# Rigelyon/ThatsMyFace

Hardware: AMD Instinct MI355X
Metric: Mpixels/s embed+extract, 4K RGB batch, 1/2/4/8 MI355X; % HBM roofline (higher is better)
Workload: dtype f64+f32 (u8 I/O)

## Files before the change

thatsmyface_amd/csrc/tmfwm_internal.h:

```cpp
#pragma once
#include <hip/hip_runtime.h>
#include <stdint.h>

#include <vector>

#include "../../include/tmfwm.h"
#include "tmfwm_sizes.h"
#include "tmfwm_tile_plan.h"

namespace tmf {

constexpr uint32_t kListShards = 2048, kShardStride = 16;

__host__ __device__ inline uint32_t shard_base(uint32_t s, uint32_t rows, uint32_t nbw)
{
    const uint32_t q = rows / kListShards, r = rows % kListShards;
    return (uint32_t)(((uint64_t)s * q + (s < r ? s : r)) * nbw);
}

struct EmbedArgs {
    const uint8_t *src;
    uint8_t *dst;
    const uint8_t *wm;
    int64_t wm_stride;
    int64_t nframes;
    int64_t frame_stride;
    int H, W, block, nbh, nbw, strips_per_row;
    int aligned;
    double alpha;
    uint32_t *fb_list;
    uint32_t *fb_count;
    uint32_t *fb_bad;
    uint32_t *slow_list;
    uint32_t *slow_count;
    uint32_t *slow_shards;
    float *key_out;
    int64_t key_stride;
};

struct ExtractArgs {
    const uint8_t *wsrc;
    const uint8_t *osrc;
    uint8_t *out;
    int64_t nframes;
    int64_t frame_stride;
    int64_t tile_stride;
    int H, W, block, nbh, nbw, strips_per_row;
    int aligned;
    float alpha32;
    uint32_t *fb_list;
    uint32_t *fb_count;
    uint32_t *fb_bad;
    uint32_t *slow_list;
    uint32_t *slow_count;
    uint32_t *slow_shards;
};

struct KeyedArgs {
    const uint8_t *src;
    const float *key;
    float *key_out;
    uint8_t *out;
    int64_t nframes;
    int64_t frame_stride;
    int64_t tile_stride;
    int64_t key_stride;
    int H, W, block, nbh, nbw, strips_per_row;
    int aligned;
    float alpha32;
    uint32_t *fb_list;
    uint32_t *fb_count;
    uint32_t *fb_bad;
    uint32_t *slow_list;
    uint32_t *slow_count;
    uint32_t *slow_shards;
};

struct EdgeArgs {
    const uint8_t *src;
    uint8_t *dst;
    int64_t frame_stride;
    int H, W, core_h, core_w, edge_w;
};

int report(int code, const char *fmt, ...);
void clear_error();
int check_frames(int64_t n, int32_t H, int32_t W, int64_t stride, int32_t block);

int64_t count_chunks(int64_t nframes, int H, int W, int block);
int embed_device_async(const uint8_t *src, int64_t n, int H, int W, int64_t stride, const uint8_t *tile, int64_t tile_stride,
                       int block, double alpha, uint8_t *dst, hipStream_t st, uint32_t *sink, int route = TMFWM_ROUTE_HYBRID);
int extract_device_async(const uint8_t *wsrc, const uint8_t *osrc, int64_t n, int H, int W, int64_t stride, int block,
                         double alpha, uint8_t *out, hipStream_t st, uint32_t *sink, int route = TMFWM_ROUTE_HYBRID);
int sum_sink(const uint32_t *sink, int64_t nchunks, int64_t *lapack);


constexpr int64_t kMaxGridY = 65535;

template <class Launch>
inline hipError_t for_frame_slices(int64_t nframes, Launch launch)
{
    for (int64_t f0 = 0; f0 < nframes; f0 += kMaxGridY) launch(f0, nframes - f0 < kMaxGridY ? nframes - f0 : kMaxGridY);
    return hipGetLastError();
}

inline unsigned list_grid(int64_t rows) { return (unsigned)(rows < (int64_t)kListShards ? rows : (int64_t)kListShards); }

template <class Args>
inline hipError_t launch_strips(Args a, int bpw, void (*strip)(Args), void (*list)(Args), hipStream_t st)
{
    if (a.nframes > kMaxGridY) return hipErrorInvalidValue;
    a.strips_per_row = (a.nbw + bpw - 1) / bpw;
    hipLaunchKernelGGL(strip, dim3((unsigned)((int64_t)a.strips_per_row * a.nbh), (unsigned)a.nframes), dim3(64), 0, st, a);
    if (list && a.slow_list) hipLaunchKernelGGL(list, dim3(list_grid(a.nframes * a.nbh)), dim3(64), 0, st, a);
    return hipGetLastError();
}

hipError_t launch_embed(const EmbedArgs &a, hipStream_t st);
hipError_t launch_embed_key_strips(const EmbedArgs &a, hipStream_t st);
bool embed_key_fused(int block);
hipError_t launch_embed_rank1(EmbedArgs a, hipStream_t st);
bool rank1_block(int block);
bool embed_defers(int block);
hipError_t launch_edges(const uint8_t *src, uint8_t *dst, int64_t nframes, int H, int W, int64_t frame_stride, int block, hipStream_t st);
hipError_t launch_extract(const ExtractArgs &a, hipStream_t st);
hipError_t launch_rgb_to_ycbcr(const uint8_t *rgb, int64_t npix, float *ycc, hipStream_t st);
hipError_t launch_rgb_to_ycbcr_f32(const float *rgb, int64_t npix, float *ycc, hipStream_t st);
hipError_t launch_ycbcr_to_rgb(const void *ycc, int dtype, int64_t npix, uint8_t *rgb, hipStream_t st);
hipError_t launch_dct2d_blocks(float *blocks, int64_t nb, int block, int inverse, hipStream_t st);
hipError_t launch_embed_fixup(const EmbedArgs &a, const uint32_t *list, const uint32_t *count, int64_t max_entries, hipStream_t st);
hipError_t launch_extract_fixup(const ExtractArgs &a, const uint32_t *list, const uint32_t *count, int64_t max_entries, hipStream_t st);
template <int B>
hipError_t embed_fixup_b(const EmbedArgs &a, const uint32_t *list, const uint32_t *count, int64_t max_entries, hipStream_t st);
template <int B>
hipError_t embed_key_fixup_b(const EmbedArgs &a, const uint32_t *list, const uint32_t *count, int64_t max_entries, hipStream_t st);
template <int B>
hipError_t embed_key_strips_b(const EmbedArgs &a, hipStream_t st);
template <int B>
hipError_t extract_fixup_b(const ExtractArgs &a, const uint32_t *list, const uint32_t *count, int64_t max_entries, hipStream_t st);
template <int B>
hipError_t sigma1_fixup_b(const KeyedArgs &a, const uint32_t *list, const uint32_t *count, int64_t max_entries, hipStream_t st);
template <int B>
hipError_t extract_keyed_fixup_b(const KeyedArgs &a, const uint32_t *list, const uint32_t *count, int64_t max_entries, hipStream_t st);
hipError_t launch_sigma1_map(const KeyedArgs &a, hipStream_t st);
hipError_t launch_extract_keyed(const KeyedArgs &a, hipStream_t st);
hipError_t launch_sigma1_fixup(const KeyedArgs &a, const uint32_t *list, const uint32_t *count, int64_t max_entries, hipStream_t st);
hipError_t launch_extract_keyed_fixup(const KeyedArgs &a, const uint32_t *list, const uint32_t *count, int64_t max_entries,
                                      hipStream_t st);
hipError_t launch_list_all(uint32_t *list, uint32_t *count, int64_t n, hipStream_t st);
hipError_t launch_pack_rgbx(const uint8_t *src4, int64_t sstride, uint8_t *dst3, int64_t dstride, int64_t n, int H, int W,
                            hipStream_t st);
hipError_t launch_unpack_rgbx(const uint8_t *src3, int64_t sstride, uint8_t *dst4, int64_t dstride, int64_t n, int H, int W,
                              hipStream_t st);
hipError_t launch_lapack_svd_blocks(const float *D, int64_t nb, int block, float *U, float *S, float *Vt, int want_v, int32_t *info,
                                    hipStream_t st);
hipError_t launch_lapack_nrm2(const double *x, int64_t nvec, int n, int inc, double *out, hipStream_t st);
hipError_t launch_svd_blocks(const float *D, int64_t nb, int block, float *U, float *S, float *Vt, int32_t *sweeps, hipStream_t st);
struct ResamplePlan {
    int ih = 0, iw = 0, oh = 0, ow = 0, y_first = 0, y_last = 0;
    bool need_h = false, need_v = false;
    ResampleAxis h, v;
    void build(int in_h, int in_w, int out_h, int out_w);
    int rows() const { return y_last - y_first; }
    size_t tmp_bytes() const { return need_h ? (size_t)rows() * ow : 0; }
    std::vector<int> pack() const;
};

hipError_t launch_resize_lanczos(const uint8_t *in, const ResamplePlan &plan, const int *tables, uint8_t *tmp, uint8_t *out,
                                 int ldo, hipStream_t st);
constexpr int64_t kResizeGroup = 1024;
size_t resize_tmp_bytes(const ResamplePlan &plan, int64_t n);
hipError_t launch_resize_lanczos_batch(const uint8_t *in, int64_t in_stride, int64_t n, const ResamplePlan &plan, const int *tables,
                                       uint8_t *tmp, uint8_t *out, int ldo, int64_t out_stride, hipStream_t st);
hipError_t launch_tiles_ragged(const TileJob *jobs, int64_t n, const int *tables, uint8_t *scratch, int64_t h_items,
                               int64_t v_items, hipStream_t st);
hipError_t launch_synth(uint64_t seed, int64_t frame0, int64_t nframes, int64_t frame_bytes, uint8_t *out, hipStream_t st);

}
```

thatsmyface_amd/csrc/tmfwm_kernels.hip:

```cpp
#include "tmfwm_blocks.h"
#include "tmfwm_passes.h"

namespace tmf {

extern template __global__ void embed_kernel<8, false>(EmbedArgs);
extern template __global__ void embed_kernel<8, true>(EmbedArgs);

template <int B, bool LIST = false>
__global__ __launch_bounds__(64, (B > 8 ? 2 : kExtract8Waves)) void extract_kernel(ExtractArgs a)
{
    constexpr int L = Geo<B>::L, BPW = Geo<B>::BPW, LD = B + 1;
    __shared__ float lds[BPW * B * LD];
    const int lane = threadIdx.x & 63, g = lane / L, q = lane % L;
    float *tile = lds + g * B * LD;
    if constexpr (LIST) {
        const uint32_t per_frame = (uint32_t)a.nbh * (uint32_t)a.nbw, rows = (uint32_t)a.nframes * (uint32_t)a.nbh;
        for (uint32_t s = blockIdx.x; s < kListShards; s += gridDim.x) {
          const uint32_t n = a.slow_shards[s * kShardStride], base = shard_base(s, rows, (uint32_t)a.nbw);
          if (n != 0 && lane == 0) atomicAdd(a.slow_count, n);
          for (uint32_t t0 = 0; t0 < n; t0 += BPW) {
            StripPos pos;
            pos.valid = t0 + g < n;
            const uint32_t id = pos.valid ? a.slow_list[base + t0 + g] : 0u;
            pos.frame = id / per_frame;
            const uint32_t rem = id % per_frame;
            pos.bi = (int)(rem / (uint32_t)a.nbw);
            pos.bj = (int)(rem % (uint32_t)a.nbw);
            float sw, so;
            bool ok;
            extract_sigmas<B, kListPowerIters>(a, pos, tile, q, sw, so, ok);
            if (pos.valid && q == 0) {
                if (ok) a.out[pos.frame * a.tile_stride + (int64_t)pos.bi * a.nbw + pos.bj] = extract_byte(sw, so, a.alpha32);
                else a.fb_list[atomicAdd(a.fb_count, 1u)] = id;
            }
            __syncthreads();
          }
        }
    } else {
        const StripPos pos = strip_pos<B>(a.strips_per_row, a.nbw);
        float sw, so;
        bool ok;
        extract_sigmas<B, kPowerIters>(a, pos, tile, q, sw, so, ok);
        if (!pos.valid || q != 0) return;
        const uint32_t id = (uint32_t)(((int64_t)blockIdx.y * a.nbh + pos.bi) * a.nbw + pos.bj);
        if (!ok) {
            if (a.slow_list) {
                const uint32_t row = blockIdx.y * (uint32_t)a.nbh + (uint32_t)pos.bi, s = row % kListShards;
                a.slow_list[shard_base(s, (uint32_t)a.nframes * (uint32_t)a.nbh, (uint32_t)a.nbw) +
                            atomicAdd(a.slow_shards + s * kShardStride, 1u)] = id;
            }
            else a.fb_list[atomicAdd(a.fb_count, 1u)] = id;
            return;
        }
        a.out[pos.frame * a.tile_stride + (int64_t)pos.bi * a.nbw + pos.bj] = extract_byte(sw, so, a.alpha32);
    }
}

__global__ __launch_bounds__(256) void edge_roundtrip_kernel(EdgeArgs a)
{
    edge_roundtrip_pixel(a, (int64_t)blockIdx.x * blockDim.x + threadIdx.x, blockIdx.y * a.frame_stride);
}

__global__ __launch_bounds__(256) void rgb_to_ycbcr_kernel(const uint8_t *__restrict__ rgb, int64_t npix, float *__restrict__ ycc)
{
    const int64_t p = (int64_t)blockIdx.x * blockDim.x + threadIdx.x;
    if (p >= npix) return;
    const uint32_t r = rgb[3 * p], g = rgb[3 * p + 1], b = rgb[3 * p + 2];
    float cbs, crs;
    chroma(r, g, b, cbs, crs);
    ycc[3 * p] = luma(r, g, b);
    ycc[3 * p + 1] = cbs;
    ycc[3 * p + 2] = crs;
}

__global__ __launch_bounds__(256) void rgb_to_ycbcr_f32_kernel(const float *__restrict__ rgb, int64_t npix, float *__restrict__ ycc)
{
    const int64_t p = (int64_t)blockIdx.x * blockDim.x + threadIdx.x;
    if (p >= npix) return;
    colour_fwd_f32(rgb[3 * p], rgb[3 * p + 1], rgb[3 * p + 2], ycc[3 * p], ycc[3 * p + 1], ycc[3 * p + 2]);
}

template <typename T>
__global__ __launch_bounds__(256) void ycbcr_to_rgb_kernel(const T *__restrict__ ycc, int64_t npix, uint8_t *__restrict__ rgb)
{
    const int64_t p = (int64_t)blockIdx.x * blockDim.x + threadIdx.x;
    if (p >= npix) return;
    uint32_t R8, G8, B8;
    colour_inv_t<T>(ycc[3 * p], ycc[3 * p + 1], ycc[3 * p + 2], R8, G8, B8);
    rgb[3 * p] = (uint8_t)R8;
    rgb[3 * p + 1] = (uint8_t)G8;
    rgb[3 * p + 2] = (uint8_t)B8;
}

template <int B, bool INVERSE>
__global__ __launch_bounds__(64) void dct2d_blocks_kernel(float *blocks, int64_t nblocks)
{
    constexpr int L = Geo<B>::L, R = Geo<B>::R, BPW = Geo<B>::BPW, LD = B + 1;
    __shared__ float lds[BPW * B * LD];
    const int lane = threadIdx.x & 63, g = lane / L, q = lane % L;
    const int64_t blk = (int64_t)blockIdx.x * BPW + g;
    const bool valid = blk < nblocks;
    float x[R][B];
#pragma unroll
    for (int r = 0; r < R; ++r)
#pragma unroll
        for (int c = 0; c < B; ++c) x[r][c] = valid && real_row<B>(q, r) ? blocks[blk * B * B + (q * R + r) * B + c] : 0.0f;
    dct2d_rows_layout<B, INVERSE>(x, lds + g * B * LD, q);
    if (valid)
#pragma unroll
        for (int r = 0; r < R; ++r)
            if (real_row<B>(q, r))
#pragma unroll
                for (int c = 0; c < B; ++c) blocks[blk * B * B + (q * R + r) * B + c] = x[r][c];
}

template <int B>
__global__ __launch_bounds__(64) void svd_blocks_kernel(const float *__restrict__ D, int64_t nblocks, float *__restrict__ U,
                                                        float *__restrict__ S, float *__restrict__ Vt, int32_t *__restrict__ sweeps)
{
    constexpr int L = Geo<B>::L, R = Geo<B>::R, BPW = Geo<B>::BPW;
    constexpr int SD = (kScratchFloats<B, L> + 1) / 2;
    __shared__ double norms[BPW * SD];
    const int lane = threadIdx.x & 63, g = lane / L, q = lane % L;
    const int64_t blk = (int64_t)blockIdx.x * BPW + g;
    const bool valid = blk < nblocks;
    float x[R][B];
#pragma unroll
    for (int r = 0; r < R; ++r)
#pragma unroll
        for (int c = 0; c < B; ++c) x[r][c] = valid && real_row<B>(q, r) ? D[blk * B * B + (q * R + r) * B + c] : 0.0f;
    double A[R][B], V[R][B];
    int nsw = svd3<B, L>(x, A, V, q, NoStamp{}, norms + g * SD);
    double sig[B];
    float Uf[R][B], Vf[R][B];
#pragma unroll
    for (int k = 0; k < B; ++k) sig[k] = cdot_part<R, B>(A, k, k);
#pragma unroll
    for (int k = 0; k < B; ++k) {
        sig[k] = __builtin_sqrt(group_sum<L>(sig[k]));
        const double inv = 1.0 / sig[k];
#pragma unroll
        for (int r = 0; r < R; ++r) {
            Uf[r][k] = sig[k] == 0.0 ? 0.0f : (float)(A[r][k] * inv);
            Vf[r][k] = (float)V[r][k];
        }
    }
    bool zero = true;
#pragma unroll
    for (int k = 0; k < B; ++k) zero = zero && (sig[k] == 0.0);
    if (zero) {
        nsw = 0;
#pragma unroll
        for (int r = 0; r < R; ++r)
#pragma unroll
            for (int k = 0; k < B; ++k) Uf[r][k] = Vf[r][k] = (q * R + r == k) ? 1.0f : 0.0f;
    }
#pragma unroll
    for (int round = 0; round < B; ++round)
#pragma unroll
        for (int k = round & 1; k + 1 < B; k += 2) {
            const bool sw = sig[k] < sig[k + 1];
            const double s0 = sig[k], s1 = sig[k + 1];
            sig[k] = sw ? s1 : s0;
            sig[k + 1] = sw ? s0 : s1;
#pragma unroll
            for (int r = 0; r < R; ++r) {
                const float u0 = Uf[r][k], u1 = Uf[r][k + 1], v0 = Vf[r][k], v1 = Vf[r][k + 1];
                Uf[r][k] = sw ? u1 : u0;
                Uf[r][k + 1] = sw ? u0 : u1;
                Vf[r][k] = sw ? v1 : v0;
                Vf[r][k + 1] = sw ? v0 : v1;
            }
        }
    if (!valid) return;
#pragma unroll
    for (int r = 0; r < R; ++r)
        if (real_row<B>(q, r))
#pragma unroll
            for (int k = 0; k < B; ++k) {
                U[blk * B * B + (q * R + r) * B + k] = Uf[r][k];
                Vt[blk * B * B + k * B + q * R + r] = Vf[r][k];
            }
    if (q == 0) {
#pragma unroll
        for (int k = 0; k < B; ++k) S[blk * B + k] = (float)sig[k];
        if (sweeps) sweeps[blk] = nsw;
    }
}

TMF_DEVI uint64_t splitmix64(uint64_t x)
{
    x += 0x9E3779B97F4A7C15ULL;
    x = (x ^ (x >> 30)) * 0xBF58476D1CE4E5B9ULL;
    x = (x ^ (x >> 27)) * 0x94D049BB133111EBULL;
    return x ^ (x >> 31);
}

__global__ __launch_bounds__(256) void synth_kernel(uint64_t seed, int64_t frame0, int64_t frame_bytes, uint8_t *out)
{
    const int64_t f = blockIdx.y;
    const uint64_t fs = seed ^ ((uint64_t)(frame0 + f) << 40);
    uint8_t *o = out + f * frame_bytes;
    for (int64_t i4 = ((int64_t)blockIdx.x * blockDim.x + threadIdx.x) * 4; i4 < frame_bytes; i4 += (int64_t)gridDim.x * blockDim.x * 4) {
        if (i4 + 4 <= frame_bytes && ((reinterpret_cast<uintptr_t>(o + i4) & 3) == 0)) {
            uint32_t w = 0;
#pragma unroll
            for (int k = 0; k < 4; ++k) w |= (uint32_t)(splitmix64(fs ^ (uint64_t)(i4 + k)) & 0xFF) << (8 * k);
            *reinterpret_cast<uint32_t *>(o + i4) = w;
        } else {
            for (int64_t i = i4; i < i4 + 4 && i < frame_bytes; ++i) o[i] = (uint8_t)(splitmix64(fs ^ (uint64_t)i) & 0xFF);
        }
    }
}

bool embed_defers(int block)
{
    return block_value(block, false, [](auto b) { return kDeferMax<b()> > 0; });
}

bool embed_key_fused(int block)
{
    return block_value(block, false, [](auto b) { return kEmbedKeyFused<b()>; });
}

hipError_t launch_embed_key_strips(const EmbedArgs &a, hipStream_t st)
{
    return for_block(a.block, [&](auto b) { return embed_key_strips_b<b()>(a, st); });
}

hipError_t launch_embed(const EmbedArgs &a, hipStream_t st)
{
    if (a.nbh > 0 && a.nbw > 0) {
        const hipError_t e = a.key_out ? launch_embed_key_strips(a, st) : for_block(a.block, [&](auto b) {
            constexpr int B = b();
            void (*list)(EmbedArgs) = nullptr;
            if constexpr (kDeferMax<B> > 0) list = embed_kernel<B, true>;
            return launch_strips(a, Geo<B>::BPW, embed_kernel<B, false>, list, st);
        });
        if (e != hipSuccess) return e;
    }
    return launch_edges(a.src, a.dst, a.nframes, a.H, a.W, a.frame_stride, a.block, st);
}

hipError_t launch_edges(const uint8_t *src, uint8_t *dst, int64_t nframes, int H, int W, int64_t frame_stride, int block, hipStream_t st)
{
    EdgeArgs e;
    e.src = src;
    e.dst = dst;
    e.H = H;
    e.W = W;
    e.frame_stride = frame_stride;
    e.core_h = (H / block) * block;
    e.core_w = (W / block) * block;
    e.edge_w = W - e.core_w;
    const int64_t n = (int64_t)e.core_h * e.edge_w + (int64_t)(H - e.core_h) * W;
    if (n == 0) return hipSuccess;
    return for_frame_slices(nframes, [&](int64_t f0, int64_t nf) {
        EdgeArgs c = e;
        c.src = src + f0 * frame_stride;
        c.dst = dst + f0 * frame_stride;
        hipLaunchKernelGGL(edge_roundtrip_kernel, dim3((unsigned)((n + 255) / 256), (unsigned)nf), dim3(256), 0, st, c);
    });
}

hipError_t launch_extract(const ExtractArgs &a, hipStream_t st)
{
    if (a.nbh == 0 || a.nbw == 0) return hipSuccess;
    return for_block(a.block, [&](auto b) {
        return launch_strips(a, Geo<b()>::BPW, extract_kernel<b(), false>, extract_kernel<b(), true>, st);
    });
}

hipError_t launch_rgb_to_ycbcr(const uint8_t *rgb, int64_t npix, float *ycc, hipStream_t st)
{
    if (npix == 0) return hipSuccess;
    hipLaunchKernelGGL(rgb_to_ycbcr_kernel, dim3((unsigned)((npix + 255) / 256)), dim3(256), 0, st, rgb, npix, ycc);
    return hipGetLastError();
}

hipError_t launch_rgb_to_ycbcr_f32(const float *rgb, int64_t npix, float *ycc, hipStream_t st)
{
    if (npix == 0) return hipSuccess;
    hipLaunchKernelGGL(rgb_to_ycbcr_f32_kernel, dim3((unsigned)((npix + 255) / 256)), dim3(256), 0, st, rgb, npix, ycc);
    return hipGetLastError();
}

hipError_t launch_ycbcr_to_rgb(const void *ycc, int dtype, int64_t npix, uint8_t *rgb, hipStream_t st)
{
    if (npix == 0) return hipSuccess;
    const dim3 grid((unsigned)((npix + 255) / 256));
    switch (dtype) {
    case TMFWM_DT_F16:
        hipLaunchKernelGGL(ycbcr_to_rgb_kernel<_Float16>, grid, dim3(256), 0, st, static_cast<const _Float16 *>(ycc), npix, rgb);
        break;
    case TMFWM_DT_F32:
        hipLaunchKernelGGL(ycbcr_to_rgb_kernel<float>, grid, dim3(256), 0, st, static_cast<const float *>(ycc), npix, rgb);
        break;
    case TMFWM_DT_F64:
        hipLaunchKernelGGL(ycbcr_to_rgb_kernel<double>, grid, dim3(256), 0, st, static_cast<const double *>(ycc), npix, rgb);
        break;
    default: return hipErrorInvalidValue;
    }
    return hipGetLastError();
}

hipError_t launch_dct2d_blocks(float *blocks, int64_t nb, int block, int inverse, hipStream_t st)
{
    if (nb == 0) return hipSuccess;
    return for_block(block, [&](auto b) {
        constexpr int B = b();
        const unsigned grid = (unsigned)((nb + Geo<B>::BPW - 1) / Geo<B>::BPW);
        if (inverse) hipLaunchKernelGGL((dct2d_blocks_kernel<B, true>), dim3(grid), dim3(64), 0, st, blocks, nb);
        else hipLaunchKernelGGL((dct2d_blocks_kernel<B, false>), dim3(grid), dim3(64), 0, st, blocks, nb);
        return hipGetLastError();
    });
}

hipError_t launch_svd_blocks(const float *D, int64_t nb, int block, float *U, float *S, float *Vt, int32_t *sweeps, hipStream_t st)
{
    if (nb == 0) return hipSuccess;
    return for_block(block, [&](auto b) {
        constexpr int B = b();
        const unsigned grid = (unsigned)((nb + Geo<B>::BPW - 1) / Geo<B>::BPW);
        hipLaunchKernelGGL(svd_blocks_kernel<B>, dim3(grid), dim3(64), 0, st, D, nb, U, S, Vt, sweeps);
        return hipGetLastError();
    });
}

#ifdef TMF_STAMPS
extern "C" int tmfwm_debug_stamps(unsigned long long *out, int reset)
{
    if (hipMemcpyFromSymbol(out, HIP_SYMBOL(g_stamps), sizeof(unsigned long long) * 16) != hipSuccess) return -5;
    if (reset) {
        unsigned long long z[16] = {};
        if (hipMemcpyToSymbol(HIP_SYMBOL(g_stamps), z, sizeof z) != hipSuccess) return -5;
    }
    return 0;
}
#endif

hipError_t launch_synth(uint64_t seed, int64_t frame0, int64_t nframes, int64_t frame_bytes, uint8_t *out, hipStream_t st)
{
    if (nframes == 0 || frame_bytes == 0) return hipSuccess;
    const int64_t per = (frame_bytes + 1023) / 1024;
    const unsigned gx = (unsigned)(per < 4096 ? per : 4096);
    return for_frame_slices(nframes, [&](int64_t f0, int64_t nf) {
        hipLaunchKernelGGL(synth_kernel, dim3(gx, (unsigned)nf), dim3(256), 0, st, seed, frame0 + f0, frame_bytes, out + f0 * frame_bytes);
    });
}

}
```

Baseline: 61370.

## Add certified fast extract path skipping DCT via luma power iteration bounds

Measured after the change: 59440. 3.1% lower.

```diff
diff --git a/thatsmyface_amd/csrc/tmfwm_dct_fwd_bounds.h b/thatsmyface_amd/csrc/tmfwm_dct_fwd_bounds.h
--- /dev/null
+++ b/thatsmyface_amd/csrc/tmfwm_dct_fwd_bounds.h
@@ -0,0 +1,9 @@
+#pragma once
+
+namespace tmf {
+
+constexpr double kDctFwdNorm = 0x1.bbba0818587b5p+5;
+constexpr double kDctCLo = 0x1.fffffd31d7e06p-1;
+constexpr double kDctCHi = 0x1.ffffff37fbb6dp-1;
+
+}
diff --git a/thatsmyface_amd/csrc/tmfwm_extract_fast.h b/thatsmyface_amd/csrc/tmfwm_extract_fast.h
--- /dev/null
+++ b/thatsmyface_amd/csrc/tmfwm_extract_fast.h
@@ -0,0 +1,142 @@
+#pragma once
+#include <stdint.h>
+
+#include "tmfwm_dct_fwd_bounds.h"
+
+#if defined(__HIPCC__)
+#include <hip/hip_runtime.h>
+#define TMF_XF_FN __host__ __device__ __forceinline__
+#else
+#define TMF_XF_FN inline
+#endif
+
+namespace tmf {
+namespace xf {
+
+constexpr float kFastLumaR = 0x1.33606ep-10f;
+constexpr float kFastLumaG = 0x1.2db8fcp-9f;
+constexpr float kFastLumaB = 0x1.d4c67p-12f;
+constexpr double kLumaErr = 0x1p-23;
+constexpr int kFastPowerIters = 2;
+constexpr float kFastAlphaMin = 0.1f;
+
+constexpr double kFastR = 0x1p-24 * kDctFwdNorm * (1.0 + 0x1p-40);
+constexpr double kFastEY = 8.0 * kLumaErr;
+
+TMF_XF_FN float luma_fast(uint32_t R, uint32_t G, uint32_t B)
+{
+    return __builtin_fmaf(kFastLumaB, (float)B, __builtin_fmaf(kFastLumaR, (float)R, kFastLumaG * (float)G));
+}
+
+template <int R, class Sum>
+TMF_XF_FN void sigma1_interval(const float (&y)[R][8], const float (&v)[8], Sum sum, double &slo, double &shi, double &F, bool &gap_pos)
+{
+    constexpr double u = 1.1102230246251565e-16;
+    double Fp = 0.0;
+#pragma unroll
+    for (int r = 0; r < R; ++r)
+#pragma unroll
+        for (int j = 0; j < 8; ++j) Fp = __builtin_fma((double)y[r][j], (double)y[r][j], Fp);
+    F = sum(Fp);
+    double vd[8], nv = 0.0;
+#pragma unroll
+    for (int j = 0; j < 8; ++j) {
+        vd[j] = (double)v[j];
+        nv = __builtin_fma(vd[j], vd[j], nv);
+    }
+    double ud[R], ap = 0.0;
+#pragma unroll
+    for (int r = 0; r < R; ++r) {
+        double acc = 0.0;
+#pragma unroll
+        for (int j = 0; j < 8; ++j) acc = __builtin_fma((double)y[r][j], vd[j], acc);
+        ud[r] = acc;
+        ap = __builtin_fma(acc, acc, ap);
+    }
+    const double rho = sum(ap) / nv;
+    double rn2 = 0.0;
+#pragma unroll
+    for (int j = 0; j < 8; ++j) {
+        double acc = 0.0;
+#pragma unroll
+        for (int r = 0; r < R; ++r) acc = __builtin_fma((double)y[r][j], ud[r], acc);
+        const double rj = sum(acc) - rho * vd[j];
+        rn2 = __builtin_fma(rj, rj, rn2);
+    }
+    const double rr0 = __builtin_sqrt(rn2 / nv) * (1.0 + 16.0 * u) + 256.0 * u * F;
+    const double rr = rr0 * rr0;
+    const double rlo = rho * (1.0 - 256.0 * u);
+    const double fhi = F * (1.0 + 256.0 * u);
+    const double gap = (rlo + rlo) - fhi;
+    const double hi = (rho + rr / (gap > 0.0 ? gap : 1.0)) * (1.0 + 256.0 * u);
+    slo = __builtin_sqrt(rlo) * (1.0 - 512.0 * u);
+    shi = __builtin_sqrt(hi) * (1.0 + 512.0 * u);
+    gap_pos = gap > 0.0 && rho == rho;
+}
+
+TMF_XF_FN void widen(double slo, double shi, double F, float &lo, float &hi)
+{
+    constexpr double u = 1.1102230246251565e-16;
+    const double r = kFastR * (__builtin_sqrt(F) + kFastEY), pad = 32.0 * u * shi;
+    const double l = (kDctCLo * (slo - kFastEY) - r - pad) * (1.0 - 512.0 * u);
+    const double h = (kDctCHi * (shi + kFastEY) + r + pad) * (1.0 + 512.0 * u);
+    lo = F == 0.0 ? 0.0f : (float)(l > 0.0 ? l : 0.0);
+    hi = F == 0.0 ? 0.0f : (float)h;
+}
+
+TMF_XF_FN uint8_t byte_of(float sw, float so, float alpha32)
+{
+    const float e = (sw - so) / alpha32;
+    double d = (double)e;
+    d = d < 0.0 ? 0.0 : d;
+    d = d > 1.0 ? 1.0 : d;
+    return (uint8_t)(uint32_t)(d * 255.0);
+}
+
+template <int R, class SumF, class SumD>
+TMF_XF_FN bool decide_block(const float (&y)[2][R][8], float alpha32, SumF sumf, SumD sumd, uint8_t &byte)
+{
+    float v[2][8];
+#pragma unroll
+    for (int m = 0; m < 2; ++m)
+#pragma unroll
+        for (int j = 0; j < 8; ++j) v[m][j] = 1.0f;
+#pragma unroll
+    for (int it = 0; it < kFastPowerIters; ++it)
+#pragma unroll
+        for (int m = 0; m < 2; ++m) {
+            float uu[R];
+#pragma unroll
+            for (int r = 0; r < R; ++r) {
+                float acc = 0.0f;
+#pragma unroll
+                for (int j = 0; j < 8; ++j) acc = __builtin_fmaf(y[m][r][j], v[m][j], acc);
+                uu[r] = acc;
+            }
+            float w[8];
+#pragma unroll
+            for (int j = 0; j < 8; ++j) {
+                float acc = 0.0f;
+#pragma unroll
+                for (int r = 0; r < R; ++r) acc = __builtin_fmaf(y[m][r][j], uu[r], acc);
+                w[j] = sumf(acc);
+            }
+#pragma unroll
+            for (int j = 0; j < 8; ++j) v[m][j] = w[j];
+        }
+    float lo[2], hi[2];
+    bool ok = true;
+#pragma unroll
+    for (int m = 0; m < 2; ++m) {
+        double slo, shi, F;
+        bool gap_pos;
+        sigma1_interval<R>(y[m], v[m], sumd, slo, shi, F, gap_pos);
+        widen(slo, shi, F, lo[m], hi[m]);
+        ok = ok && (gap_pos || F == 0.0);
+    }
+    byte = byte_of(lo[0], hi[1], alpha32);
+    return ok && byte == byte_of(hi[0], lo[1], alpha32);
+}
+
+}
+}
diff --git a/thatsmyface_amd/csrc/tmfwm_extract_fast.hip b/thatsmyface_amd/csrc/tmfwm_extract_fast.hip
--- /dev/null
+++ b/thatsmyface_amd/csrc/tmfwm_extract_fast.hip
@@ -0,0 +1,96 @@
+#include <cmath>
+#include <cstdlib>
+
+#include "tmfwm_blocks.h"
+#include "tmfwm_extract_fast.h"
+#include "tmfwm_passes.h"
+
+namespace tmf {
+
+constexpr int kExtractFastWaves = 3;
+
+__global__ __launch_bounds__(64, kExtractFastWaves) void extract_fast_kernel(ExtractArgs a)
+{
+    constexpr int B = 8, L = Geo<B>::L, R = Geo<B>::R;
+    const int lane = threadIdx.x & 63, q = lane % L;
+    const StripPos pos = strip_pos<B>(a.strips_per_row, a.nbw);
+    float y[2][R][B];
+    {
+        uint32_t w[2][R][Geo<B>::NW];
+        load_block_rows<B>(a.wsrc + pos.frame * a.frame_stride, a.W, pos, q, a.aligned, w[0]);
+        load_block_rows<B>(a.osrc + pos.frame * a.frame_stride, a.W, pos, q, a.aligned, w[1]);
+#pragma unroll
+        for (int m = 0; m < 2; ++m)
+#pragma unroll
+            for (int r = 0; r < R; ++r)
+#pragma unroll
+                for (int c = 0; c < B; ++c)
+                    y[m][r][c] = xf::luma_fast(byte_at(w[m][r], 3 * c), byte_at(w[m][r], 3 * c + 1), byte_at(w[m][r], 3 * c + 2));
+    }
+    uint8_t byte;
+    const bool ok = xf::decide_block<R>(
+        y, a.alpha32, [](float v) { return group_sum<L>(v); }, [](double v) { return group_sum<L>(v); }, byte);
+    const bool lead = pos.valid && q == 0;
+    if (lead && ok) a.out[pos.frame * a.tile_stride + (int64_t)pos.bi * a.nbw + pos.bj] = byte;
+    const bool app = lead && !ok;
+    const unsigned long long mask = __ballot(app);
+    if (mask == 0) return;
+    const uint32_t row = blockIdx.y * (uint32_t)a.nbh + (uint32_t)pos.bi, s = row % kListShards;
+    const int first = __ffsll(mask) - 1;
+    uint32_t slot = 0;
+    if (lane == first) slot = atomicAdd(a.slow_shards + s * kShardStride, (uint32_t)__popcll(mask));
+    slot = (uint32_t)__shfl((int)slot, first) + (uint32_t)__popcll(mask & ((1ull << lane) - 1ull));
+    if (app)
+        a.slow_list[shard_base(s, (uint32_t)a.nframes * (uint32_t)a.nbh, (uint32_t)a.nbw) + slot] =
+            (uint32_t)(((int64_t)blockIdx.y * a.nbh + pos.bi) * a.nbw + pos.bj);
+}
+
+bool extract_fast_applies(const ExtractArgs &a)
+{
+    if (a.block != 8 || !a.slow_list || !a.slow_shards) return false;
+    if (!std::isfinite(a.alpha32) || !(std::fabs(a.alpha32) >= xf::kFastAlphaMin)) return false;
+    const char *e = std::getenv("TMFWM_EXTRACT_FAST");
+    return !(e && *e == '0');
+}
+
+constexpr unsigned kFastListSlices = 8;
+
+__global__ __launch_bounds__(64, kExtract8Waves) void extract_fast_list_kernel(ExtractArgs a)
+{
+    constexpr int B = 8, L = Geo<B>::L, BPW = Geo<B>::BPW, LD = B + 1;
+    __shared__ float lds[BPW * B * LD];
+    const int lane = threadIdx.x & 63, g = lane / L, q = lane % L;
+    float *tile = lds + g * B * LD;
+    const uint32_t per_frame = (uint32_t)a.nbh * (uint32_t)a.nbw, rows = (uint32_t)a.nframes * (uint32_t)a.nbh;
+    const uint32_t s = blockIdx.x;
+    const uint32_t n = a.slow_shards[s * kShardStride], base = shard_base(s, rows, (uint32_t)a.nbw);
+    if (blockIdx.y == 0 && n != 0 && lane == 0) atomicAdd(a.slow_count, n);
+    for (uint32_t t0 = blockIdx.y * BPW; t0 < n; t0 += gridDim.y * BPW) {
+        StripPos pos;
+        pos.valid = t0 + g < n;
+        const uint32_t id = pos.valid ? a.slow_list[base + t0 + g] : 0u;
+        pos.frame = id / per_frame;
+        const uint32_t rem = id % per_frame;
+        pos.bi = (int)(rem / (uint32_t)a.nbw);
+        pos.bj = (int)(rem % (uint32_t)a.nbw);
+        float sw, so;
+        bool ok;
+        extract_sigmas<B, kListPowerIters>(a, pos, tile, q, sw, so, ok);
+        if (pos.valid && q == 0) {
+            if (ok) a.out[pos.frame * a.tile_stride + (int64_t)pos.bi * a.nbw + pos.bj] = extract_byte(sw, so, a.alpha32);
+            else a.fb_list[atomicAdd(a.fb_count, 1u)] = id;
+        }
+        __syncthreads();
+    }
+}
+
+hipError_t launch_extract_fast(ExtractArgs a, hipStream_t st)
+{
+    if (a.nframes > kMaxGridY) return hipErrorInvalidValue;
+    a.strips_per_row = (a.nbw + Geo<8>::BPW - 1) / Geo<8>::BPW;
+    hipLaunchKernelGGL(extract_fast_kernel, dim3((unsigned)((int64_t)a.strips_per_row * a.nbh), (unsigned)a.nframes), dim3(64), 0, st, a);
+    hipLaunchKernelGGL(extract_fast_list_kernel, dim3(list_grid(a.nframes * a.nbh), kFastListSlices), dim3(64), 0, st, a);
+    return hipGetLastError();
+}
+
+}
diff --git a/thatsmyface_amd/csrc/tmfwm_internal.h b/thatsmyface_amd/csrc/tmfwm_internal.h
--- a/thatsmyface_amd/csrc/tmfwm_internal.h
+++ b/thatsmyface_amd/csrc/tmfwm_internal.h
@@ -124,6 +124,8 @@
 bool embed_defers(int block);
 hipError_t launch_edges(const uint8_t *src, uint8_t *dst, int64_t nframes, int H, int W, int64_t frame_stride, int block, hipStream_t st);
 hipError_t launch_extract(const ExtractArgs &a, hipStream_t st);
+bool extract_fast_applies(const ExtractArgs &a);
+hipError_t launch_extract_fast(ExtractArgs a, hipStream_t st);
 hipError_t launch_rgb_to_ycbcr(const uint8_t *rgb, int64_t npix, float *ycc, hipStream_t st);
 hipError_t launch_rgb_to_ycbcr_f32(const float *rgb, int64_t npix, float *ycc, hipStream_t st);
 hipError_t launch_ycbcr_to_rgb(const void *ycc, int dtype, int64_t npix, uint8_t *rgb, hipStream_t st);
diff --git a/thatsmyface_amd/csrc/tmfwm_kernels.hip b/thatsmyface_amd/csrc/tmfwm_kernels.hip
--- a/thatsmyface_amd/csrc/tmfwm_kernels.hip
+++ b/thatsmyface_amd/csrc/tmfwm_kernels.hip
@@ -266,6 +266,7 @@
 hipError_t launch_extract(const ExtractArgs &a, hipStream_t st)
 {
     if (a.nbh == 0 || a.nbw == 0) return hipSuccess;
+    if (extract_fast_applies(a)) return launch_extract_fast(a, st);
     return for_block(a.block, [&](auto b) {
         return launch_strips(a, Geo<b()>::BPW, extract_kernel<b(), false>, extract_kernel<b(), true>, st);
     });
```
